# jmschrei/PyPore

Measured on AMD Instinct MI355X. Metric: Msamples/sec segmented (SpeedyStatSplit, 10^8-sample trace); %HBM roofline, higher is better.
Workload: dtype int32/f64 (exact integer block sums of fp32 or int16 samples; decisions in fp64)

## Files before the change

### pypore_amd/csrc/poreseg.hip

```cpp
#include <hip/hip_runtime.h>

#include <algorithm>
#include <chrono>
#include <complex>
#include <cmath>
#include <cstdarg>
#include <cstdio>
#include <cstdlib>
#include <cstring>
#include <initializer_list>
#include <condition_variable>
#include <mutex>
#include <string>
#include <thread>
#include <tuple>
#include <type_traits>
#include <vector>

#include "poreseg.h"
#include "seg_device.hpp"
#include "seg_align.hpp"
#include "seg_pairwise.hpp"
#include "seg_hmm.hpp"

// ... 73 lines not shown
    bool defer_sync = false;
    int scan_lds_pad = 0;
    int k0_unaligned = 1;
    int single_pass = 1;
    int gather_fused = 1;
    int download_by_kernel = 1;
    int debug = 0;
#ifdef PS_DIAG
    int dbg_phase = 0;
    int dbg_k0_nogrp = 0;
#endif
    int k0_shared = 0;
    hipEvent_t ev_front[2] = {};
    bool stream_idle = true;
    int tree_par = 1;
    int groups = 1;
    int scan_bs = 1;
    int wide_bs = 1;
    int bridge_single = 1 << 30;
    int tree_tail_pct = 0;
    int slots_pct = 100;
    int tree_jobs_per_wave = 4;
    int tree_screen = 1;
    struct OccKey { const void *fn; int nt; size_t lds; int per_cu; };
    std::vector<OccKey> occ_cache;
    std::vector<std::pair<const void *, int>> attr_cache;
    struct TileCache {
        bool valid = false;
        int32_t n_ev = 0; int mw = 0, W = 0; int64_t L = 0; bool use_bs = false;
        std::vector<int64_t> ev_start, ev_len;
        size_t nj = 0, jb = 0, up_bytes = 0; int64_t list_entries = 0, total_len = 0, sample_end = 0, nb_total = 0;
    } tile_cache;
    DevBuf bsum, ev_info, chunk_mabs, ev_boff, blk_mm, grp, filt_fwd, filt_agg, filt_zin, up_dev;
    DevBuf align_in, align_scratch;
    DevBuf pw_in, pw_scratch;
    long long pw_budget = 2ll << 30;
    DevBuf ev_info_tr;
    DevBuf blk_cls, cls_mm;
    DevBuf pre_c;
    DevBuf nt_log;
    int64_t nt_cap = 65536, nt_hdr_cap = -1;
    int64_t nt_seen = -1, nt_call_cap = 0;
    std::vector<int64_t> nt_ev_start, nt_ev_len;
    DevBuf hmm_model, hmm_off, hmm_bp, hmm_last, hmm_flags;
    std::vector<char> hmm_blob;
    long long hmm_bp_budget = 512ll << 20;
    DevBuf hmm_fmat, hmm_acc, hmm_skip;
    DevBuf hmm_pmax;
    DevBuf hmm_samp;
    long long hmm_fb_budget = 4ll << 30;
    bool hmm_expect_lds = true;
    int stitch_host = 0;
    DevBuf ev_len, det_counts, det_tics, det_cand;
    DevBuf bridges, bmeta, tile_i32, sp_off, spine_items, asm_hdr, ev_first_tile;
    DevBuf bridge_ext, ext_slot, ext_list;
    DevBuf lat_state, lat_seam, lat_res;
    unsigned lat_tag_next = 1;
    unsigned lat_tag_base = 0;
    int lat_help = 1;
    int bridge_budget = BR_MAX;
    int bridge_ext_on = 1;
    HostBuf h_hdr;
    DevBuf spine_jobs, spine_scratch, spine_dense, spine_meta, tree_jobs, tree_scratch, tree_spill, tree_defer, screen_acc,
        tree_counts, items, item_pos, first_item, ev_off, bounds_off, small;
    HostBuf h_meta, h_dense, h_small, h_up;
    hipEvent_t ev[10] = {};
    int timing = 1;
    double ms[8] = {0, 0, 0, 0, 0, 0, 0, 0};
    int64_t counters[16] = {0, 0, 0, 0, 0, 0, 0, 0, 0, 0, 0, 0, 0, 0, -1, -1};
    bool screen_ran = false;
};

namespace {

int fail(ps_ctx *ctx, int code, const char *fmt, ...)
{
    if (ctx) {
        char buf[512];
        va_list ap;
        va_start(ap, fmt);
        vsnprintf(buf, sizeof buf, fmt, ap);
        va_end(ap);
        ctx->err = buf;
    }
    return code;
}

#define HIP_TRY(ctx, expr)                                                                        \
    do {                                                                                          \
        hipError_t e_ = (expr);                                                                   \
        if (e_ != hipSuccess)                                                                     \
            return fail(ctx, PS_ERR_HIP, "%s failed: %s (%s:%d)", #expr, hipGetErrorString(e_), __FILE__, __LINE__); \
    } while (0)
// ... 36 lines not shown
        c.made = true;
    }
    const unsigned long long t = c.next++;
    *ticket = t;
    const int m = std::min(max_in_flight, K0Chain::RING / 2);
    if (t >= static_cast<unsigned long long>(m)) {
        const unsigned long long w = t - static_cast<unsigned long long>(m);
        if (c.gen[w % K0Chain::RING] == w + 1) HIP_TRY(ctx, hipStreamWaitEvent(st, c.ev[w % K0Chain::RING], 0));
    }
    return PS_OK;
}
int chain_publish(ps_ctx *ctx, int device, hipStream_t st, unsigned long long ticket)
{
    K0Chain &c = g_chain[device & 15];
    std::lock_guard<std::mutex> lk(c.mu);
    HIP_TRY(ctx, hipEventRecord(c.ev[ticket % K0Chain::RING], st));
    c.gen[ticket % K0Chain::RING] = ticket + 1;
    return PS_OK;
}
constexpr size_t SMALL_TAIL = 64 * 1024;
struct SmallLayout { unsigned long long status, work0, work1, work2, dense, stamp[12], life[9], qctl, qhead, tree_tail; AsmHeader hdr;
                     unsigned long long lat_ctl[6]; int lat_prog[LAT_D];
                     unsigned long long nt_cur;
                     unsigned long long tree_defer[3]; };

int make_cfg(ps_ctx *ctx, const void *d_samples, const ps_sample_format *fmt, int mw, int maxw, int W,
             double min_gain, DevCfg *c)
{
    if (!fmt) return fail(ctx, PS_ERR_ARG, "sample format is NULL");
    if (fmt->dtype != PS_DTYPE_F32 && fmt->dtype != PS_DTYPE_I16)
        return fail(ctx, PS_ERR_ARG, "unknown dtype %d", fmt->dtype);
    if (!(fmt->quantum > 0) || !std::isfinite(fmt->quantum))
        return fail(ctx, PS_ERR_ARG, "quantum must be positive and finite");
    c->samples = d_samples;
    c->dtype = fmt->dtype;
    c->off_counts = fmt->dtype == PS_DTYPE_F32 ? 0 : fmt->offset_counts;
    c->dc_counts = fmt->dtype == PS_DTYPE_F32 ? static_cast<double>(fmt->offset_counts) : 0.0;
    c->noise_k = ctx->noise_k;
    c->inv_q = static_cast<float>(1.0 / fmt->quantum);
    c->q = fmt->quantum;
    c->q2 = fmt->quantum * fmt->quantum;
    c->mw = mw; c->maxw = maxw; c->W = W; c->half = W / 2;
    c->min_gain = min_gain;
    c->mode = ctx->mode;
    c->prune = ctx->prune;
    c->lds_cap = std::max(1, std::min(W, ctx->lds_max_samples));
    c->bsum = nullptr; c->ev_info = nullptr; c->chunk_tot = nullptr; c->blk_mm = nullptr; c->grp = nullptr; c->bs_wide = 0;
// ... 453 lines not shown
    float ms = 0;
    if (ctx->timing >= 2 && hipEventElapsedTime(&ms, ctx->ev[2], ctx->ev[3]) == hipSuccess) ctx->ms[1] = ms;
    if (ctx->timing >= 2 && hipEventElapsedTime(&ms, ctx->ev[3], ctx->ev[4]) == hipSuccess) ctx->ms[2] = ms;
    ctx->ms[3] = std::chrono::duration<double, std::milli>(std::chrono::steady_clock::now() - t_begin).count();
    return PS_OK;
}



LatHelp lat_help_of(ps_ctx *ctx, const DevCfg &cfg, SmallLayout *sm)
{
    if (!ctx->lat_help || cfg.bsum == nullptr || !ctx->lat_res.p) return LAT_NONE;
    LatHelp h;
    h.ctl = sm->lat_ctl;
    h.state = ctx->lat_state.as<unsigned long long>();
    h.seam = ctx->lat_seam.as<int>();
    h.prog = sm->lat_prog;
    h.res = ctx->lat_res.as<unsigned long long>();
    h.tag_base = ctx->lat_tag_base;
    h.stay = ctx->lat_help == 2 ? 1 : 0;
    return h;
}

template <int DT> int launch_bridge_la(ps_ctx *ctx, const DevCfg &cfg, unsigned nj, SmallLayout *sm)
{
    const unsigned grid = std::min(nj, resident_slots(ctx, bridge_la_kernel<DT>, 64 * BR_LA, 0));
    hipLaunchKernelGGL((bridge_la_kernel<DT>), dim3(grid), dim3(64 * BR_LA), 0, ctx->stream, cfg,
                       ctx->spine_jobs.as<SpineJob>(), ctx->spine_scratch.as<int2>(), ctx->spine_meta.as<int4>(),
                       ctx->bridges.as<int2>(), ctx->bmeta.as<int4>(), reinterpret_cast<unsigned *>(&sm->status),
                       &sm->work0, static_cast<int>(nj), nullptr, nullptr, nullptr, 0, ctx->bridge_budget, static_cast<int>(EXT_MAX),
                       lat_help_of(ctx, cfg, sm));
    HIP_TRY(ctx, hipGetLastError());
    return PS_OK;
}

template <int NT, int DT> int launch_bridge(ps_ctx *ctx, const DevCfg &cfg, unsigned nj, SmallLayout *sm)
{
    ScanShape s;
    if (int rc = scan_shape<NT>(ctx, bridge_kernel<NT, DT>, cfg, nj, &s)) return rc;
    hipLaunchKernelGGL((bridge_kernel<NT, DT>), dim3(s.grid), dim3(NT), s.lds, ctx->stream, cfg,
                       ctx->spine_jobs.as<SpineJob>(), ctx->spine_scratch.as<int2>(), ctx->spine_meta.as<int4>(),
                       ctx->bridges.as<int2>(), ctx->bmeta.as<int4>(), reinterpret_cast<unsigned *>(&sm->status),
                       &sm->work0, static_cast<int>(nj), ctx->bridge_single, ctx->bridge_budget,
                       NT == 64 ? lat_help_of(ctx, cfg, sm) : LAT_NONE);
    HIP_TRY(ctx, hipGetLastError());
    return PS_OK;
}

void reset_call_stats(ps_ctx *ctx)
{
    for (double &m : ctx->ms) m = 0;
    for (int64_t &c : ctx->counters) c = 0;
    ctx->counters[14] = ctx->counters[15] = -1;
    ctx->screen_ran = false;
}

int reserve_items(ps_ctx *ctx, int64_t items_cap, int64_t total_len, int mw)
{
    const size_t n = static_cast<size_t>(std::max<int64_t>(1, items_cap));
    const size_t tscratch_bound = static_cast<size_t>(total_len / mw + items_cap + 1);
    HIP_TRY(ctx, ctx->spine_items.reserve(n * sizeof(int4)));
    HIP_TRY(ctx, ctx->tree_jobs.reserve(n * sizeof(TreeJob)));
    HIP_TRY(ctx, ctx->tree_counts.reserve((n + (static_cast<size_t>(items_cap) >> GS_LOG) + 2) * sizeof(int32_t)));
    HIP_TRY(ctx, ctx->items.reserve(n * sizeof(Item)));
    HIP_TRY(ctx, ctx->item_pos.reserve((static_cast<size_t>(items_cap) + 1) * sizeof(int64_t)));
    HIP_TRY(ctx, ctx->tree_scratch.reserve(tscratch_bound * sizeof(int32_t)));
    HIP_TRY(ctx, ctx->tree_spill.reserve(tscratch_bound * sizeof(int2)));
    if (ctx->tree_screen) {
        HIP_TRY(ctx, ctx->tree_defer.reserve(n * sizeof(int2)));
        HIP_TRY(ctx, ctx->screen_acc.reserve_zeroed(static_cast<size_t>(SCREEN_ACC) * SCREEN_ACC_STRIDE * sizeof(unsigned long long), ctx->stream));
    }
    return PS_OK;
}

struct DigestWant { bool wide = false, grp = false, blk_mm = false, cls = false; };
int reserve_digest(ps_ctx *ctx, int64_t nb_pad, int32_t n_ev, const DigestWant &want)
{
// ... 53 lines not shown
    }
    bool queued = skip_k0;
#ifdef PS_DIAG
    if constexpr (!(FLAGS & DT_WIDE)) {
        if (!queued && ns == 3) { enqueue_k0<FLAGS, 3, 6>(ctx, cfg, st, k, k0_grid, k0_grp); queued = true; }
        if (!queued && ns == 4) { enqueue_k0<FLAGS, 4, 8>(ctx, cfg, st, k, k0_grid, k0_grp); queued = true; }
    }
#endif
    if (!queued) enqueue_k0<FLAGS, 2, 2>(ctx, cfg, st, k, k0_grid, k0_grp);
    HIP_TRY(ctx, hipGetLastError());
    return PS_OK;
}
int k0_done(ps_ctx *ctx, hipStream_t st)
{
    if (!ctx->chain_held) return PS_OK;
    ctx->chain_held = false;
    return chain_publish(ctx, ctx->device, st, ctx->chain_ticket);
}

template <int FLAGS> int launch_scans_bs(ps_ctx *ctx, const DevCfg &cfg, unsigned nj, SmallLayout *sm)
{
    if (int rc = by_dtype<FLAGS>(cfg.dtype, [&](auto dt) { return launch_spine<64, dt()>(ctx, cfg, nj, sm, true); })) return rc;
    if (ctx->timing >= 2) HIP_TRY(ctx, hipEventRecord(ctx->ev[6], ctx->stream));
    if (int rc = by_dtype<FLAGS>(cfg.dtype, [&](auto dt) { return launch_bridge<64, dt()>(ctx, cfg, nj, sm); })) return rc;
    return by_dtype<FLAGS>(cfg.dtype, [&](auto dt) { return launch_bridge_la<dt()>(ctx, cfg, nj, sm); });
}

int device_stitch_batch_(ps_ctx *ctx, const DevCfg &cfg_in, int bs_mode, const int64_t *ev_start, const int64_t *ev_len, int32_t n_ev, int mw, int W,
                        int32_t *d_bounds, int64_t cap, int64_t *h_bounds_off, ps_segstat *d_stats,
                        std::chrono::steady_clock::time_point t_begin, bool digest_ready = false)
{
    DevCfg cfg = cfg_in;
    const bool use_bs = bs_mode != 0;
    const bool wide = bs_mode == 2;
    cfg.bs_wide = wide ? 1 : 0;
    int64_t L = ctx->tile_len;
    ps_ctx::TileCache &tc = ctx->tile_cache;
    const size_t evb = (static_cast<size_t>(n_ev) + 1) * sizeof(int64_t);
    bool reuse = tc.valid && tc.n_ev == n_ev && tc.mw == mw && tc.W == W && tc.L == L && tc.use_bs == use_bs &&
                 std::equal(ev_start, ev_start + n_ev, tc.ev_start.begin()) && std::equal(ev_len, ev_len + n_ev, tc.ev_len.begin());
    if (!reuse) {
        tc.valid = false;
        int64_t total_len = 0, sample_end = 0;
        for (int e = 0; e < n_ev; ++e) { total_len += ev_len[e]; sample_end = std::max(sample_end, ev_start[e] + ev_len[e]); }
        int64_t Lt = L;
        if (Lt <= 0) Lt = use_bs ? ((total_len + 4095) / 4096 >= 8LL * W ? (total_len + 4095) / 4096
                                                                         : std::max<int64_t>(4LL * W, (total_len + 1535) / 1536))
                                 : std::max<int64_t>(8LL * W, (total_len + 1023) / 1024);
// ... 39 lines not shown
    }
    const size_t nj = tc.nj, jb = tc.jb, up_bytes = tc.up_bytes;
    const int64_t list_entries = tc.list_entries, total_len = tc.total_len, sample_end = tc.sample_end;
    ctx->counters[2] = static_cast<int64_t>(nj);
    const int64_t max_items = list_entries + static_cast<int64_t>(nj) * BR_MAX;

    HIP_TRY(ctx, ctx->spine_scratch.reserve(std::max<int64_t>(1, list_entries) * sizeof(int2)));
    HIP_TRY(ctx, ctx->spine_meta.reserve(std::max<size_t>(4, nj) * sizeof(int4)));
    HIP_TRY(ctx, ctx->bridges.reserve(std::max<size_t>(1, nj) * BR_MAX * sizeof(int2)));
    if (use_bs && ctx->lat_help) {
        const size_t res_bytes = static_cast<size_t>(LAT_D) * LAT_C * sizeof(unsigned long long);
        HIP_TRY(ctx, ctx->lat_state.reserve(LAT_D * sizeof(unsigned long long)));
        HIP_TRY(ctx, ctx->lat_seam.reserve(LAT_D * sizeof(int)));
        HIP_TRY(ctx, ctx->lat_res.reserve_zeroed(res_bytes, ctx->stream));
        if (ctx->lat_tag_next + 2u * LAT_TAGS >= (1u << 24)) {
            HIP_TRY(ctx, hipMemsetAsync(ctx->lat_res.p, 0, res_bytes, ctx->stream));
            ctx->stream_idle = false;
            ctx->lat_tag_next = 1;
        }
        ctx->lat_tag_base = ctx->lat_tag_next;
        ctx->lat_tag_next += LAT_TAGS;
    }
    HIP_TRY(ctx, ctx->bmeta.reserve(std::max<size_t>(1, nj) * sizeof(int4)));
    HIP_TRY(ctx, ctx->tile_i32.reserve(std::max<size_t>(1, nj) * 4 * sizeof(int)));
    HIP_TRY(ctx, ctx->sp_off.reserve((nj + 1) * sizeof(long long)));
    if (int irc = reserve_items(ctx, max_items, total_len, mw)) return irc;
    HIP_TRY(ctx, ctx->first_item.reserve(evb));
    if (evb <= SMALL_TAIL) ctx->bounds_off.alias(ctx->small.as<char>() + sizeof(SmallLayout));
    else HIP_TRY(ctx, ctx->bounds_off.reserve(evb));
    ctx->asm_hdr.alias(&ctx->small.as<SmallLayout>()->hdr);
    HIP_TRY(ctx, ctx->h_small.reserve(sizeof(SmallLayout)));
    FrontStream *front = (ctx->k0_shared && use_bs && tc.nj) ? front_for(ctx) : nullptr;
    hipStream_t fs = front ? front->s : ctx->stream;
    std::unique_lock<std::mutex> front_lock;
    if (front) {
        front_lock = std::unique_lock<std::mutex>(front->mu);
        if (!ctx->stream_idle) {
            HIP_TRY(ctx, hipEventRecord(ctx->ev_front[0], ctx->stream));
            HIP_TRY(ctx, hipStreamWaitEvent(fs, ctx->ev_front[0], 0));
        }
    }
    {
        const char *up = ctx->h_up.as<char>();
        void *up_devptr = nullptr;
        if (ctx->upload_by_kernel && hipHostGetDevicePointer(&up_devptr, const_cast<char *>(up), 0) != hipSuccess) { up_devptr = nullptr; (void)hipGetLastError(); }
        if (up_devptr) {
// ... 121 lines not shown
            for (size_t g = 0; g < nj; ++g) n_fail += h_bm[g].w == BR_FAIL_REACHED || (h_bm[g].w == BR_FAIL && h_bm[g].x == ctx->bridge_budget);
            ext_stride = n_fail <= static_cast<size_t>(EXT_SLOTS) ? EXT_MAX : EXT_MAX_MANY;
        }
        const int slot_cap = EXT_SLOTS * (EXT_MAX / ext_stride);
        for (size_t g = 0; g < nj; ++g) {
            const bool reached = h_bm[g].w == BR_FAIL_REACHED;
            const bool gave_up = h_bm[g].x == ctx->bridge_budget;
            if (!reached && !(h_bm[g].w == BR_FAIL && gave_up)) continue;
            const bool open_tile = h_mt[g].x == 0 && h_bm[g].x == 0;
            if (!gave_up && !open_tile) { if (reached) hopeless = true; continue; }
            if (slots_used + static_cast<int>(list.size()) < slot_cap) list.push_back(static_cast<int>(g));
            else if (reached) hopeless = true;
        }
        if (list.empty() || hopeless) break;
        if (ctx->debug) fprintf(stderr, "[poreseg] second chance, round %d: %zu seams continued on the device\n", round + 1, list.size());
        const size_t n_ext = list.size();
        HIP_TRY(ctx, ctx->bridge_ext.reserve(static_cast<size_t>(EXT_SLOTS) * EXT_MAX * sizeof(int2)));
        HIP_TRY(ctx, ctx->ext_slot.reserve(nj * sizeof(int)));
        HIP_TRY(ctx, ctx->ext_list.reserve(static_cast<size_t>(EXT_SLOTS) * (EXT_MAX / EXT_MAX_MANY) * sizeof(int)));
        HIP_TRY(ctx, hipMemcpyAsync(ctx->ext_list.p, list.data(), n_ext * sizeof(int), hipMemcpyHostToDevice, ctx->stream));
        HIP_TRY(ctx, hipStreamSynchronize(ctx->stream));
        HIP_TRY(ctx, hipMemsetAsync(&sm->hdr, 0, sizeof(AsmHeader), ctx->stream));
        if (ctx->tree_screen) HIP_TRY(ctx, hipMemsetAsync(&sm->tree_defer[0], 0, sizeof sm->tree_defer[0], ctx->stream));
        {
            const unsigned g = static_cast<unsigned>(n_ext);
            auto extend = [&](auto dt) {
                hipLaunchKernelGGL((bridge_la_kernel<dt(), true>), dim3(g), dim3(64 * BR_LA), 0, ctx->stream, cfg,
                                   ctx->spine_jobs.as<SpineJob>(), ctx->spine_scratch.as<int2>(), ctx->spine_meta.as<int4>(),
                                   ctx->bridges.as<int2>(), ctx->bmeta.as<int4>(), reinterpret_cast<unsigned *>(&sm->status),
                                   &sm->work0, static_cast<int>(n_ext), ctx->ext_list.as<int>(), ctx->bridge_ext.as<int2>(),
                                   ctx->ext_slot.as<int>(), slots_used, BR_MAX, ext_stride);
            };
            if (wide) by_dtype<DT_WIDE>(cfg.dtype, extend);
            else by_dtype(cfg.dtype, extend);
            HIP_TRY(ctx, hipGetLastError());
        }
        ctx->counters[4] += static_cast<int64_t>(n_ext);
        slots_used += static_cast<int>(n_ext);
        items_cap += static_cast<int64_t>(n_ext) * ext_stride;
        if (int irc = reserve_items(ctx, items_cap, total_len, mw)) return irc;
    }
    ctx->counters[3] = hd.n_items;
    float ms = 0;
    if (ctx->timing >= 2 && nj && hipEventElapsedTime(&ms, ctx->ev[7], ctx->ev[0]) == hipSuccess) ctx->ms[6] = ms;
    if (ctx->timing >= 2 && nj && hipEventElapsedTime(&ms, ctx->ev[0], ctx->ev[6]) == hipSuccess) ctx->ms[0] = ms;
    if (ctx->timing >= 2 && nj && hipEventElapsedTime(&ms, ctx->ev[6], ctx->ev[1]) == hipSuccess) ctx->ms[5] = ms;
    if (ctx->timing >= 2 && hipEventElapsedTime(&ms, ctx->ev[1], ctx->ev[5]) == hipSuccess) ctx->ms[4] = ms;
    return rc;
}
int device_stitch_batch(ps_ctx *ctx, const DevCfg &cfg_in, int bs_mode, const int64_t *ev_start, const int64_t *ev_len, int32_t n_ev, int mw, int W,
                        int32_t *d_bounds, int64_t cap, int64_t *h_bounds_off, ps_segstat *d_stats,
                        std::chrono::steady_clock::time_point t_begin, bool digest_ready = false)
{
    const int rc = device_stitch_batch_(ctx, cfg_in, bs_mode, ev_start, ev_len, n_ev, mw, W, d_bounds, cap, h_bounds_off, d_stats, t_begin, digest_ready);
    ctx->chain_held = false;
    return rc;
}
}

namespace {
std::mutex g_probe_mu;
int g_unaligned_ok[16] = {-1, -1, -1, -1, -1, -1, -1, -1, -1, -1, -1, -1, -1, -1, -1, -1};
int k0_unaligned_probe(int device, hipStream_t st)
{
    std::lock_guard<std::mutex> lk(g_probe_mu);
// ... 98 lines not shown
        if (hipEventCreateWithFlags(&e, hipEventDisableTiming) != hipSuccess) { delete ctx; return PS_ERR_HIP; }
    if (ctx->small.reserve(sizeof(SmallLayout) + SMALL_TAIL) != hipSuccess) { delete ctx; return PS_ERR_HIP; }
    ctx->lds_max_samples = (LDS_BYTES_MAX - 1024 * 8 - 256) / (static_cast<int>(sizeof(lds_t)) + 1);
    ctx->k0_unaligned = k0_unaligned_probe(device, ctx->stream);
#ifdef PS_DIAG
    diag_env(ctx);
#endif
    *out = ctx;
    return PS_OK;
}

void ps_destroy(ps_ctx *ctx)
{
    if (!ctx) return;
    (void)hipSetDevice(ctx->device);
    (void)hipStreamSynchronize(ctx->stream);
    DevBuf *bufs[] = {&ctx->spine_jobs, &ctx->spine_scratch, &ctx->spine_dense, &ctx->spine_meta, &ctx->tree_jobs,
                      &ctx->tree_scratch, &ctx->tree_spill, &ctx->tree_defer, &ctx->screen_acc, &ctx->tree_counts, &ctx->items, &ctx->item_pos,
                      &ctx->first_item, &ctx->ev_off, &ctx->bounds_off, &ctx->small, &ctx->bridges, &ctx->bmeta,
                      &ctx->tile_i32, &ctx->sp_off, &ctx->spine_items, &ctx->asm_hdr, &ctx->ev_first_tile, &ctx->ev_len,
                      &ctx->det_counts, &ctx->det_tics, &ctx->det_cand, &ctx->bsum, &ctx->ev_info, &ctx->chunk_mabs,
                      &ctx->ev_boff, &ctx->blk_mm, &ctx->grp, &ctx->filt_fwd, &ctx->filt_agg, &ctx->filt_zin, &ctx->up_dev,
                      &ctx->align_in, &ctx->align_scratch, &ctx->pw_in, &ctx->pw_scratch, &ctx->bridge_ext, &ctx->ext_slot, &ctx->ext_list,
                      &ctx->lat_state, &ctx->lat_seam, &ctx->lat_res, &ctx->pre_c, &ctx->ev_info_tr, &ctx->blk_cls,
                      &ctx->cls_mm, &ctx->nt_log, &ctx->hmm_model, &ctx->hmm_off, &ctx->hmm_bp,
                      &ctx->hmm_last, &ctx->hmm_flags, &ctx->hmm_fmat, &ctx->hmm_acc, &ctx->hmm_skip, &ctx->hmm_pmax,
                      &ctx->hmm_samp};
    for (DevBuf *b : bufs) b->release();
    ctx->h_meta.release(); ctx->h_dense.release(); ctx->h_small.release(); ctx->h_up.release(); ctx->h_hdr.release();
    for (auto &e : ctx->ev) if (e) (void)hipEventDestroy(e);
    for (auto &e : ctx->ev_front) if (e) (void)hipEventDestroy(e);
    if (ctx->own_stream) (void)hipStreamDestroy(ctx->stream);
    delete ctx;
}

const char *ps_last_error(const ps_ctx *ctx) { return ctx ? ctx->err.c_str() : "null context"; }

int ps_set_tiling(ps_ctx *ctx, int64_t tile_len, int64_t halo)
{
    if (!ctx || tile_len < 0 || halo < 0) return PS_ERR_ARG;
    ctx->tile_len = tile_len;
    ctx->halo = halo;
    return PS_OK;
}

#ifdef PS_DIAG
static int diag_mask_stream(ps_ctx *ctx, hipStream_t *st, int first, int count, int stride, bool invert)
// ... 30 lines not shown
    else if (n == "k0_waves" && value >= 0 && value <= 16) ctx->k0_waves = static_cast<int>(value);
    else if (n == "k0_shared") ctx->k0_shared = value != 0;
    else if (n == "k0_admit" && value >= 0) ctx->k0_admit = static_cast<int>(value);
    else if (n == "bridge_ext" && (value == 0 || value == 1)) ctx->bridge_ext_on = static_cast<int>(value);
    else if (n == "lat_help" && value >= 0 && value <= 2) ctx->lat_help = static_cast<int>(value);
    else if (n == "shared_device" && value >= 0 && value <= 4096) {
        const bool sh = value > 1;
        ctx->k0_waves = sh ? 1 : 0;
        ctx->lat_help = sh ? 0 : 1;
        ctx->k0_admit = value > 3 ? 3 : 0;
    }
    else if (n == "hmm_bp_budget" && value >= 1) ctx->hmm_bp_budget = value;
    else if (n == "hmm_fb_budget" && value >= 1) ctx->hmm_fb_budget = value;
    else if (n == "pairwise_budget" && value >= 1) ctx->pw_budget = value;
    else if (n == "hmm_expect_lds") ctx->hmm_expect_lds = value != 0;
    else if (n == "single_pass") ctx->single_pass = value != 0;
    else if (n == "gather_fused") ctx->gather_fused = value != 0;
    else if (n == "download_by_kernel") ctx->download_by_kernel = value != 0;
    else if (n == "debug") ctx->debug = value != 0;
    else if (n == "k0_unaligned") ctx->k0_unaligned = value != 0 ? k0_unaligned_probe(ctx->device, ctx->stream) : 0;
    else if (n == "slots_pct" && value >= 1 && value <= 100) ctx->slots_pct = static_cast<int>(value);
    else if (n == "tree_jobs_per_wave" && value >= 0 && value <= 1024) ctx->tree_jobs_per_wave = static_cast<int>(value);
    else if (n == "tree_screen") ctx->tree_screen = value != 0;
    else if (n == "noise_k_ppm" && value >= 0) ctx->noise_k = static_cast<float>(static_cast<double>(value) * 1.0e-6);
#ifdef PS_DIAG
    else if (n == "dbg_phase" && value >= 0 && value <= 2) ctx->dbg_phase = static_cast<int>(value);
    else if (n == "dbg_k0_nogrp") ctx->dbg_k0_nogrp = value != 0;
    else if (n == "cu_mask" && ctx->own_stream)
        return diag_mask_stream(ctx, &ctx->stream, static_cast<int>(value & 0xfff), static_cast<int>((value >> 12) & 0xfff),
                                static_cast<int>((value >> 24) & 0xff), ((value >> 32) & 1) != 0);
    else if (n == "k0_sets" && value >= 2 && value <= 4) ctx->k0_sets = static_cast<int>(value);
    else if (n == "scan_lds_pad" && value >= 0 && value <= 65536) ctx->scan_lds_pad = static_cast<int>(value);
    else if (n == "rep_eval" && value >= 1) ctx->rep_eval = static_cast<int>(value);
    else if (n == "rep_stage" && value >= 1) ctx->rep_stage = static_cast<int>(value);
    else if (n == "rep_sum" && value >= 1) ctx->rep_sum = static_cast<int>(value);
#endif
    else if (n == "bridge_budget" && value >= 1 && value <= BR_MAX) ctx->bridge_budget = static_cast<int>(value);
    else if (n == "wide_bs") { ctx->wide_bs = value != 0; ctx->wide_skip = 0; }
    else if (n == "bridge_single" && value >= 1) ctx->bridge_single = static_cast<int>(value);
    else if (n == "tree_tail_pct" && value >= 0 && value <= 100) ctx->tree_tail_pct = static_cast<int>(value);
    else if (n == "filter_fused") ctx->filter_fused = value != 0;
    else if (n == "upload_by_kernel") ctx->upload_by_kernel = value != 0;
    else if (n == "timing") ctx->timing = static_cast<int>(std::max<int64_t>(0, std::min<int64_t>(2, value)));
    else if (n == "tree_mw") ctx->tree_mw = value != 0;
    else if (n == "spine_nt" && (value == 256 || value == 512 || value == 1024)) ctx->spine_nt = static_cast<int>(value);
    else if (n == "tree_nt" && (value == 256 || value == 512)) ctx->tree_nt = static_cast<int>(value);
// ... 1711 lines not shown
```

### pypore_amd/csrc/seg_device.hpp

```cpp
#pragma once
#include <hip/hip_runtime.h>
#include <stdint.h>
#include "poreseg.h"

namespace ps {

constexpr int LDS_STACK = 128;
constexpr int MAX_WAVES = 16;
constexpr int OBUF = 256;
constexpr int BR_MAX = 256;
constexpr int LST_MAX = 256;
constexpr int LAT_D = 256;
constexpr int LAT_W = 16;
constexpr int LAT_C = 2048;
constexpr int LAT_TAGS = 4096;
struct LatHelp {
    unsigned long long *ctl;
    unsigned long long *state;
    int *seam;
    int *prog;
    unsigned long long *res;
    unsigned tag_base;
    int stay;
};
// ... 1162 lines not shown
            if (threadIdx.x == 0) {
                unsigned long long pos = atomicAdd(dense_count, static_cast<unsigned long long>(cnt));
                meta[jb] = make_int4(cnt, ended, static_cast<int>(pos), 0);
                sh.bcast = static_cast<int>(pos);
            }
            __syncthreads();
            const int pos = sh.bcast;
            for (int i = threadIdx.x; i < cnt; i += NT) dense[pos + i] = i < flushed ? out[i] : sh.obuf[i - flushed];
        }
        __syncthreads();
    }
    flush(bad, wk, status, work, 0);
}

enum : int { BR_NONE = 0, BR_JOINED = 1, BR_ENDED = 2, BR_FAIL = 3, BR_DEFER = 4,
              BR_FAIL_REACHED = 5 };
__device__ __forceinline__ int2 bridge_at(const int2 *bridges, const int2 *ext, const int *ext_slot, int ext_stride, int g, int i)
{
    return i < BR_MAX ? bridges[static_cast<long long>(g) * BR_MAX + i]
                      : ext[static_cast<long long>(ext_slot[g]) * ext_stride + (i - BR_MAX)];
}
constexpr int BR_PATIENCE = 3;

template <int NT, int DT>
__global__ __launch_bounds__(NT, (NT == 64 ? PS_BRIDGE_MINW : 4)) PS_BRIDGE_REGS void bridge_kernel(DevCfg c, const SpineJob *jobs, const int2 *lists,
                                                       const int4 *meta, int2 *bridges, int4 *bmeta,
                                                       unsigned *status, unsigned long long *work, int n_jobs, int max_single,
                                                       int budget = BR_MAX,
                                                       LatHelp lat = LAT_NONE)
{
    extern __shared__ int ys[];
    __shared__ SharedT<NT> sh;
    if (c.bsum != nullptr && (*status & ST_WIDE_RANGE) != 0u) return;
    unsigned bad = 0;
    Work wk = PS_WORK_INIT;
    for (int g = blockIdx.x; g < n_jobs; g += gridDim.x) {
        const SpineJob job = jobs[g];
        const int4 m = meta[g];
        const bool last_tile = (g - job.first_tile) == job.ntiles - 1;
        if (last_tile || m.y != 0) {
            if (threadIdx.x == 0) bmeta[g] = make_int4(0, -1, 0, BR_NONE);
            continue;
        }
        if (m.x == 0 && g != job.first_tile) {
            if (threadIdx.x == 0) bmeta[g] = make_int4(0, -1, 0, BR_FAIL);
            continue;
        }
        int a = m.x > 0 ? lists[job.out_off + m.x - 1].x : job.start;
        int cnt = 0, st = BR_FAIL, jt = -1, ji = 0, cached = -1, ccnt = 0;
        const EvRef er = ev_ref_of(c, job.ev);
        for (int step = 0; step <= budget; ++step) {
            int u = a / job.tile_len;
            if (u > job.ntiles - 1) u = job.ntiles - 1;
            u += job.first_tile;
            const SpineJob uj = jobs[u];
            if (u != cached) {
                ccnt = meta[u].x;
                __syncthreads();
                for (int i = threadIdx.x; i < ccnt && i < SharedT<NT>::LN; i += NT) sh.lst[i] = lists[uj.out_off + i].x;
// ... 29 lines not shown
            bmeta[g] = make_int4(cnt, jt, ji, st);
            if (st == BR_DEFER && lat.ctl != nullptr && c.half > 0) {
                const long long ps0 = static_cast<long long>(a) + static_cast<long long>(jt + LAT_W) * c.half;
                if (ps0 < static_cast<long long>(job.end) - 2LL * c.mw) {
                    int u = static_cast<int>(ps0 / job.tile_len);
                    if (u > job.ntiles - 1) u = job.ntiles - 1;
                    const int4 mu = meta[job.first_tile + u];
                    if (mu.x == 0 && mu.y == 0) atomicAdd(&lat.ctl[0], 1ull);
                }
            }
        }
        __syncthreads();
    }
    flush(bad, wk, status, work, 1);
}

constexpr int BR_LA = 4;
template <int DT, bool EXT = false>
__global__ __launch_bounds__(64 * BR_LA, PS_BRIDGE_MINW) PS_BRIDGE_REGS void bridge_la_kernel(DevCfg c, const SpineJob *jobs, const int2 *lists,
                                                                  const int4 *meta, int2 *bridges, int4 *bmeta,
                                                                  unsigned *status, unsigned long long *work, int n_jobs,
                                                                  const int *ext_list = nullptr, int2 *ext = nullptr, int *ext_slot = nullptr,
                                                                  int slot_base = 0, int budget = BR_MAX, int ext_stride = EXT_MAX,
                                                                  LatHelp lat = LAT_NONE)
{
    __shared__ unsigned long long lat_e;
    __shared__ unsigned long long lat_state[EXT ? 1 : LAT_D];
    __shared__ int lat_prog[EXT ? 1 : LAT_D];
    __shared__ SharedT<64> shw[BR_LA];
    __shared__ int lst[LST_MAX];
    __shared__ int2 obuf[BR_MAX];
    __shared__ int2 res[BR_LA];
    if ((*status & ST_WIDE_RANGE) != 0u) return;
    const bool lat_stay = !EXT && lat.res != nullptr && c.half > 0 && (lat.ctl[0] != 0ull || lat.stay != 0);
    const int wave = __builtin_amdgcn_readfirstlane(static_cast<int>(threadIdx.x >> 6));
    SharedT<64> &sh = shw[wave];
    unsigned bad = 0;
    Work wk = PS_WORK_INIT;
    enum : int { O_CONT = 0, O_HIT = 1, O_EARLY = 2, O_LATE = 3, O_NONE = 4 };
    const int LIMIT = EXT ? BR_MAX + ext_stride : budget;
    for (int gi = blockIdx.x; gi < n_jobs; gi += gridDim.x) {
        const int g = EXT ? ext_list[gi] : gi;
        const int4 bm = bmeta[g];
        if (!EXT && bm.w != BR_DEFER) continue;
        const SpineJob job = jobs[g];
        const int4 m = meta[g];
        int cnt = bm.x;
        for (int i = threadIdx.x; i < cnt && i < BR_MAX; i += 64 * BR_LA) obuf[i] = bridges[static_cast<int64_t>(g) * BR_MAX + i];
        __syncthreads();
        const long long slot = slot_base + gi;
        int a = cnt > 0 ? obuf[cnt - 1].x : (m.x > 0 ? lists[job.out_off + m.x - 1].x : job.start);
        int st = BR_FAIL, jt = -1, ji = 0, cached = -1, ccnt = 0;
        const EvRef er = ev_ref_of(c, job.ev);
        long long jres = EXT ? (cnt == 0 && m.x == 0 ? m.z : 0) : bm.y;
        const bool lat_use = lat_stay;
        int lslot = -1;
        long long la0 = 0;
        unsigned ltag = 0;
        bool lat_valid = false;
        for (int step = cnt; step <= LIMIT; ++step) {
            int u = a / job.tile_len;
            if (u > job.ntiles - 1) u = job.ntiles - 1;
            u += job.first_tile;
            const SpineJob uj = jobs[u];
            if (u != cached) {
// ... 1156 lines not shown
```

### pypore_amd/engine.py

```python
import collections
import ctypes
import os
import threading
import warnings

import numpy as np
import torch

from . import _lib

_contexts = {}

DEFAULT_OPTIONS = {}
DEFAULT_TILING = [0, 0]
POOL_OVERRIDES = {}

EVENT_CAP = 1 << 16

_ENV_OPTIONS = {
    "PORESEG_MODE": "mode", "PORESEG_SPINE_NT": "spine_nt", "PORESEG_TREE_NT": "tree_nt", "PORESEG_PRUNE": "prune",
    "PORESEG_SCAN_BS": "scan_bs", "PORESEG_GROUPS": "groups", "PORESEG_TREE_PAR": "tree_par", "PORESEG_K0_WAVES": "k0_waves",
    "PORESEG_K0_SHARED": "k0_shared", "PORESEG_K0_MAX": "k0_admit", "PORESEG_K0_SETS": "k0_sets", "PORESEG_WIDE_BS": "wide_bs",
    "PORESEG_BRIDGE_SINGLE": "bridge_single", "PORESEG_TREE_TAIL": "tree_tail_pct", "PORESEG_FILTER_FUSED": "filter_fused",
    "PORESEG_UPLOAD": "upload_by_kernel", "PORESEG_TIMING": "timing", "PORESEG_TREE_MW": "tree_mw",
    "PORESEG_TREE_JPW": "tree_jobs_per_wave", "PORESEG_TREE_SCREEN": "tree_screen", "PORESEG_SLOTS_PCT": "slots_pct", "PORESEG_BRIDGE_EXT": "bridge_ext",
    "PORESEG_LAT_HELP": "lat_help", "PORESEG_BRIDGE_BUDGET": "bridge_budget", "PORESEG_DEBUG": "debug",
    "PORESEG_GATHER_FUSED": "gather_fused", "PORESEG_SINGLE_PASS": "single_pass", "PORESEG_DOWNLOAD": "download_by_kernel", "PORESEG_K0_UNALIGNED": "k0_unaligned",
    "PORESEG_DBG_PHASE": "dbg_phase", "PORESEG_DBG_K0_NOGRP": "dbg_k0_nogrp", "PORESEG_SCAN_LDS_PAD": "scan_lds_pad", "PORESEG_REP_STAGE": "rep_stage",
}


def options_from_env(environ=None):
    env = os.environ if environ is None else environ
    opts = {}
    for var, name in _ENV_OPTIONS.items():
        if var in env and env[var] != "":
            opts[name] = int(env[var])
    if env.get("PORESEG_STITCH"):
        opts["stitch_host"] = 1 if env["PORESEG_STITCH"] == "host" else 0
    if "PORESEG_NOISE_K" in env:
        opts["noise_k_ppm"] = int(round(float(env["PORESEG_NOISE_K"]) * 1e6))
    tiling = [int(env.get("PORESEG_TILE", "0") or 0), int(env.get("PORESEG_HALO", "0") or 0)]
    pool = {}
    if "PORESEG_POOL_K0_WAVES" in env:
        pool["k0_waves"] = int(env["PORESEG_POOL_K0_WAVES"])
    if "PORESEG_POOL_K0_MAX" in env:
        pool["k0_admit"] = int(env["PORESEG_POOL_K0_MAX"])
    if env.get("PORESEG_POOL_SHARED", "0") == "1":
# ... 899 lines not shown
```

Baseline: 537,300.

## Add seam-join prepass that resolves easy tile seams before bridge kernels

Adds a lightweight seam_join_kernel that, for each tile seam, classifies it as none, failed, or directly joinable by binary-searching the next tile's split list for the current endpoint. Joined and trivial seams get their bmeta written immediately, and only unresolved seams are compacted into a list. The bridge and lookahead-bridge kernels then iterate over that compacted list instead of every job, and the bridge grid shrinks accordingly. This saves scanning work on seams that need no bridging, at the cost of an extra launch, an atomic-based compaction, and a counter reset on the extension path.

Measured after the change: 534,600. No clear change (-0.5%).

```diff
diff --git a/pypore_amd/csrc/poreseg.hip b/pypore_amd/csrc/poreseg.hip
--- a/pypore_amd/csrc/poreseg.hip
+++ b/pypore_amd/csrc/poreseg.hip
@@ -119,6 +119,7 @@
     int slots_pct = 100;
     int tree_jobs_per_wave = 4;
     int tree_screen = 1;
+    int seam_join = 1;
     struct OccKey { const void *fn; int nt; size_t lds; int per_cu; };
     std::vector<OccKey> occ_cache;
     std::vector<std::pair<const void *, int>> attr_cache;
@@ -151,6 +152,7 @@
     DevBuf ev_len, det_counts, det_tics, det_cand;
     DevBuf bridges, bmeta, tile_i32, sp_off, spine_items, asm_hdr, ev_first_tile;
     DevBuf bridge_ext, ext_slot, ext_list;
+    DevBuf seam_list;
     DevBuf lat_state, lat_seam, lat_res;
     unsigned lat_tag_next = 1;
     unsigned lat_tag_base = 0;
@@ -166,6 +168,7 @@
     double ms[8] = {0, 0, 0, 0, 0, 0, 0, 0};
     int64_t counters[16] = {0, 0, 0, 0, 0, 0, 0, 0, 0, 0, 0, 0, 0, 0, -1, -1};
     bool screen_ran = false;
+    bool join_ran = false;
 };
 
 namespace {
@@ -248,7 +251,8 @@
 struct SmallLayout { unsigned long long status, work0, work1, work2, dense, stamp[12], life[9], qctl, qhead, tree_tail; AsmHeader hdr;
                      unsigned long long lat_ctl[6]; int lat_prog[LAT_D];
                      unsigned long long nt_cur;
-                     unsigned long long tree_defer[3]; };
+                     unsigned long long tree_defer[3];
+                     unsigned long long seam_join[JOIN_CTL]; };
 
 int make_cfg(ps_ctx *ctx, const void *d_samples, const ps_sample_format *fmt, int mw, int maxw, int W,
              double min_gain, DevCfg *c)
@@ -748,29 +752,43 @@
     return h;
 }
 
-template <int DT> int launch_bridge_la(ps_ctx *ctx, const DevCfg &cfg, unsigned nj, SmallLayout *sm)
+template <int DT> int launch_bridge_la(ps_ctx *ctx, const DevCfg &cfg, unsigned nj, SmallLayout *sm, bool listed = false)
 {
     const unsigned grid = std::min(nj, resident_slots(ctx, bridge_la_kernel<DT>, 64 * BR_LA, 0));
     hipLaunchKernelGGL((bridge_la_kernel<DT>), dim3(grid), dim3(64 * BR_LA), 0, ctx->stream, cfg,
                        ctx->spine_jobs.as<SpineJob>(), ctx->spine_scratch.as<int2>(), ctx->spine_meta.as<int4>(),
                        ctx->bridges.as<int2>(), ctx->bmeta.as<int4>(), reinterpret_cast<unsigned *>(&sm->status),
-                       &sm->work0, static_cast<int>(nj), nullptr, nullptr, nullptr, 0, ctx->bridge_budget, static_cast<int>(EXT_MAX),
-                       lat_help_of(ctx, cfg, sm));
+                       &sm->work0, static_cast<int>(nj), listed ? ctx->seam_list.as<int>() : nullptr, nullptr, nullptr, 0,
+                       ctx->bridge_budget, static_cast<int>(EXT_MAX), lat_help_of(ctx, cfg, sm), listed ? &sm->seam_join[0] : nullptr);
     HIP_TRY(ctx, hipGetLastError());
     return PS_OK;
 }
 
-template <int NT, int DT> int launch_bridge(ps_ctx *ctx, const DevCfg &cfg, unsigned nj, SmallLayout *sm)
+template <int NT, int DT> int launch_bridge(ps_ctx *ctx, const DevCfg &cfg, unsigned nj, SmallLayout *sm, bool listed = false)
 {
     ScanShape s;
     if (int rc = scan_shape<NT>(ctx, bridge_kernel<NT, DT>, cfg, nj, &s)) return rc;
+    if (listed) s.grid = std::max(1u, std::min(s.grid, (nj + 3) / 4));
     hipLaunchKernelGGL((bridge_kernel<NT, DT>), dim3(s.grid), dim3(NT), s.lds, ctx->stream, cfg,
                        ctx->spine_jobs.as<SpineJob>(), ctx->spine_scratch.as<int2>(), ctx->spine_meta.as<int4>(),
                        ctx->bridges.as<int2>(), ctx->bmeta.as<int4>(), reinterpret_cast<unsigned *>(&sm->status),
                        &sm->work0, static_cast<int>(nj), ctx->bridge_single, ctx->bridge_budget,
-                       NT == 64 ? lat_help_of(ctx, cfg, sm) : LAT_NONE);
+                       NT == 64 ? lat_help_of(ctx, cfg, sm) : LAT_NONE,
+                       listed ? ctx->seam_list.as<int>() : nullptr, listed ? &sm->seam_join[0] : nullptr);
     HIP_TRY(ctx, hipGetLastError());
     return PS_OK;
+}
+
+bool launch_seam_join(ps_ctx *ctx, unsigned nj, SmallLayout *sm)
+{
+    if (!ctx->seam_join || ctx->seam_list.cap < nj * sizeof(int)) return false;
+    const unsigned grid = std::min((nj + JOIN_NT - 1) / JOIN_NT, 1024u);
+    hipLaunchKernelGGL(seam_join_kernel, dim3(grid), dim3(JOIN_NT), 0, ctx->stream, ctx->spine_jobs.as<SpineJob>(),
+                       ctx->spine_scratch.as<int2>(), ctx->spine_meta.as<int4>(), ctx->bmeta.as<int4>(),
+                       reinterpret_cast<const unsigned *>(&sm->status), static_cast<int>(nj), ctx->seam_list.as<int>(), sm->seam_join);
+    if (hipGetLastError() != hipSuccess) return false;
+    ctx->join_ran = true;
+    return true;
 }
 
 void reset_call_stats(ps_ctx *ctx)
@@ -779,6 +797,7 @@
     for (int64_t &c : ctx->counters) c = 0;
     ctx->counters[14] = ctx->counters[15] = -1;
     ctx->screen_ran = false;
+    ctx->join_ran = false;
 }
 
 int reserve_items(ps_ctx *ctx, int64_t items_cap, int64_t total_len, int mw)
@@ -878,8 +897,9 @@
 {
     if (int rc = by_dtype<FLAGS>(cfg.dtype, [&](auto dt) { return launch_spine<64, dt()>(ctx, cfg, nj, sm, true); })) return rc;
     if (ctx->timing >= 2) HIP_TRY(ctx, hipEventRecord(ctx->ev[6], ctx->stream));
-    if (int rc = by_dtype<FLAGS>(cfg.dtype, [&](auto dt) { return launch_bridge<64, dt()>(ctx, cfg, nj, sm); })) return rc;
-    return by_dtype<FLAGS>(cfg.dtype, [&](auto dt) { return launch_bridge_la<dt()>(ctx, cfg, nj, sm); });
+    const bool listed = launch_seam_join(ctx, nj, sm);
+    if (int rc = by_dtype<FLAGS>(cfg.dtype, [&](auto dt) { return launch_bridge<64, dt()>(ctx, cfg, nj, sm, listed); })) return rc;
+    return by_dtype<FLAGS>(cfg.dtype, [&](auto dt) { return launch_bridge_la<dt()>(ctx, cfg, nj, sm, listed); });
 }
 
 int device_stitch_batch_(ps_ctx *ctx, const DevCfg &cfg_in, int bs_mode, const int64_t *ev_start, const int64_t *ev_len, int32_t n_ev, int mw, int W,
@@ -965,6 +985,7 @@
         ctx->lat_tag_next += LAT_TAGS;
     }
     HIP_TRY(ctx, ctx->bmeta.reserve(std::max<size_t>(1, nj) * sizeof(int4)));
+    if (use_bs && ctx->seam_join) HIP_TRY(ctx, ctx->seam_list.reserve(std::max<size_t>(1, nj) * sizeof(int)));
     HIP_TRY(ctx, ctx->tile_i32.reserve(std::max<size_t>(1, nj) * 4 * sizeof(int)));
     HIP_TRY(ctx, ctx->sp_off.reserve((nj + 1) * sizeof(long long)));
     if (int irc = reserve_items(ctx, max_items, total_len, mw)) return irc;
@@ -1132,6 +1153,7 @@
         HIP_TRY(ctx, hipStreamSynchronize(ctx->stream));
         HIP_TRY(ctx, hipMemsetAsync(&sm->hdr, 0, sizeof(AsmHeader), ctx->stream));
         if (ctx->tree_screen) HIP_TRY(ctx, hipMemsetAsync(&sm->tree_defer[0], 0, sizeof sm->tree_defer[0], ctx->stream));
+        if (ctx->join_ran) HIP_TRY(ctx, hipMemsetAsync(&sm->seam_join[0], 0, sizeof sm->seam_join[0], ctx->stream));
         {
             const unsigned g = static_cast<unsigned>(n_ext);
             auto extend = [&](auto dt) {
@@ -1151,6 +1173,10 @@
         if (int irc = reserve_items(ctx, items_cap, total_len, mw)) return irc;
     }
     ctx->counters[3] = hd.n_items;
+    if (ctx->debug && ctx->join_ran && (rc == PS_OK || rc == RC_FALLBACK)) {
+        const unsigned long long *sj = ctx->h_small.as<SmallLayout>()->seam_join;
+        fprintf(stderr, "[poreseg] seam join: %zu seams, %llu joined, %llu none, %llu failed, %llu listed\n", nj, sj[1], sj[2], sj[3], sj[4]);
+    }
     float ms = 0;
     if (ctx->timing >= 2 && nj && hipEventElapsedTime(&ms, ctx->ev[7], ctx->ev[0]) == hipSuccess) ctx->ms[6] = ms;
     if (ctx->timing >= 2 && nj && hipEventElapsedTime(&ms, ctx->ev[0], ctx->ev[6]) == hipSuccess) ctx->ms[0] = ms;
@@ -1295,7 +1321,7 @@
                       &ctx->det_counts, &ctx->det_tics, &ctx->det_cand, &ctx->bsum, &ctx->ev_info, &ctx->chunk_mabs,
                       &ctx->ev_boff, &ctx->blk_mm, &ctx->grp, &ctx->filt_fwd, &ctx->filt_agg, &ctx->filt_zin, &ctx->up_dev,
                       &ctx->align_in, &ctx->align_scratch, &ctx->pw_in, &ctx->pw_scratch, &ctx->bridge_ext, &ctx->ext_slot, &ctx->ext_list,
-                      &ctx->lat_state, &ctx->lat_seam, &ctx->lat_res, &ctx->pre_c, &ctx->ev_info_tr, &ctx->blk_cls,
+                      &ctx->seam_list, &ctx->lat_state, &ctx->lat_seam, &ctx->lat_res, &ctx->pre_c, &ctx->ev_info_tr, &ctx->blk_cls,
                       &ctx->cls_mm, &ctx->nt_log, &ctx->hmm_model, &ctx->hmm_off, &ctx->hmm_bp,
                       &ctx->hmm_last, &ctx->hmm_flags, &ctx->hmm_fmat, &ctx->hmm_acc, &ctx->hmm_skip, &ctx->hmm_pmax,
                       &ctx->hmm_samp};
@@ -1372,6 +1398,7 @@
     else if (n == "slots_pct" && value >= 1 && value <= 100) ctx->slots_pct = static_cast<int>(value);
     else if (n == "tree_jobs_per_wave" && value >= 0 && value <= 1024) ctx->tree_jobs_per_wave = static_cast<int>(value);
     else if (n == "tree_screen") ctx->tree_screen = value != 0;
+    else if (n == "seam_join") ctx->seam_join = value != 0;
     else if (n == "noise_k_ppm" && value >= 0) ctx->noise_k = static_cast<float>(static_cast<double>(value) * 1.0e-6);
 #ifdef PS_DIAG
     else if (n == "dbg_phase" && value >= 0 && value <= 2) ctx->dbg_phase = static_cast<int>(value);
diff --git a/pypore_amd/csrc/seg_device.hpp b/pypore_amd/csrc/seg_device.hpp
--- a/pypore_amd/csrc/seg_device.hpp
+++ b/pypore_amd/csrc/seg_device.hpp
@@ -1208,19 +1208,83 @@
 }
 constexpr int BR_PATIENCE = 3;
 
+#ifndef PS_JOIN_VGPRS
+#define PS_JOIN_VGPRS 32
+#endif
+constexpr int JOIN_NT = 256;
+constexpr int JOIN_CTL = 6;
+__global__ __launch_bounds__(JOIN_NT) __attribute__((amdgpu_num_vgpr(PS_JOIN_VGPRS))) void seam_join_kernel(
+    const SpineJob *__restrict__ jobs, const int2 *__restrict__ lists, const int4 *__restrict__ meta, int4 *__restrict__ bmeta,
+    const unsigned *status, int n_jobs, int *__restrict__ seam_list, unsigned long long *ctl)
+{
+    if ((*status & ST_WIDE_RANGE) != 0u) return;
+    enum : int { J_IDLE = -1, J_LIST = -2 };
+    const int lane = static_cast<int>(threadIdx.x & 63u);
+    for (int g0 = blockIdx.x * JOIN_NT; g0 < n_jobs; g0 += gridDim.x * JOIN_NT) {
+        const int g = g0 + static_cast<int>(threadIdx.x);
+        int st = J_IDLE;
+        if (g < n_jobs) {
+            const SpineJob job = jobs[g];
+            const int4 m = meta[g];
+            const bool last_tile = (g - job.first_tile) == job.ntiles - 1;
+            if (last_tile || m.y != 0) st = BR_NONE;
+            else if (m.x == 0 && g != job.first_tile) st = BR_FAIL;
+            else {
+                const int a = m.x > 0 ? lists[job.out_off + m.x - 1].x : job.start;
+                int u = a / job.tile_len;
+                if (u > job.ntiles - 1) u = job.ntiles - 1;
+                u += job.first_tile;
+                int found = -2;
+                if (a == jobs[u].start) found = -1;
+                else {
+                    const int2 *lu = lists + jobs[u].out_off;
+                    int lo = 0, hi = meta[u].x - 1;
+                    while (lo <= hi) {
+                        const int mid = (lo + hi) >> 1;
+                        const int v = lu[mid].x;
+                        if (v == a) { found = mid; break; }
+                        if (v < a) lo = mid + 1; else hi = mid - 1;
+                    }
+                }
+                if (found != -2 && u != g) { st = BR_JOINED; bmeta[g] = make_int4(0, u, found, BR_JOINED); }
+                else st = J_LIST;
+            }
+            if (st == BR_NONE || st == BR_FAIL) bmeta[g] = make_int4(0, -1, 0, st);
+        }
+        const unsigned long long listed = __ballot(st == J_LIST);
+        const int n_joined = __popcll(__ballot(st == BR_JOINED)), n_none = __popcll(__ballot(st == BR_NONE)),
+                  n_fail = __popcll(__ballot(st == BR_FAIL)), n_list = __popcll(listed);
+        unsigned long long base = 0;
+        if (lane == 0) {
+            if (n_list) { base = atomicAdd(&ctl[0], static_cast<unsigned long long>(n_list)); atomicAdd(&ctl[4], static_cast<unsigned long long>(n_list)); }
+            if (n_joined) atomicAdd(&ctl[1], static_cast<unsigned long long>(n_joined));
+            if (n_none) atomicAdd(&ctl[2], static_cast<unsigned long long>(n_none));
+            if (n_fail) atomicAdd(&ctl[3], static_cast<unsigned long long>(n_fail));
+        }
+        if (n_list) {
+            base = __shfl(base, 0);
+            if (st == J_LIST) seam_list[base + __popcll(listed & ((1ull << lane) - 1ull))] = g;
+        }
+    }
+}
+
 template <int NT, int DT>
 __global__ __launch_bounds__(NT, (NT == 64 ? PS_BRIDGE_MINW : 4)) PS_BRIDGE_REGS void bridge_kernel(DevCfg c, const SpineJob *jobs, const int2 *lists,
                                                        const int4 *meta, int2 *bridges, int4 *bmeta,
                                                        unsigned *status, unsigned long long *work, int n_jobs, int max_single,
                                                        int budget = BR_MAX,
-                                                       LatHelp lat = LAT_NONE)
+                                                       LatHelp lat = LAT_NONE,
+                                                       const int *seam_list = nullptr, const unsigned long long *seam_count = nullptr)
 {
     extern __shared__ int ys[];
     __shared__ SharedT<NT> sh;
     if (c.bsum != nullptr && (*status & ST_WIDE_RANGE) != 0u) return;
     unsigned bad = 0;
     Work wk = PS_WORK_INIT;
-    for (int g = blockIdx.x; g < n_jobs; g += gridDim.x) {
+    const bool listed = NT == 64 && seam_list != nullptr;
+    const int n_seams = listed ? min(static_cast<int>(*seam_count), n_jobs) : n_jobs;
+    for (int gi = blockIdx.x; gi < n_seams; gi += gridDim.x) {
+        const int g = listed ? seam_list[gi] : gi;
         const SpineJob job = jobs[g];
         const int4 m = meta[g];
         const bool last_tile = (g - job.first_tile) == job.ntiles - 1;
@@ -1296,7 +1360,8 @@
                                                                   unsigned *status, unsigned long long *work, int n_jobs,
                                                                   const int *ext_list = nullptr, int2 *ext = nullptr, int *ext_slot = nullptr,
                                                                   int slot_base = 0, int budget = BR_MAX, int ext_stride = EXT_MAX,
-                                                                  LatHelp lat = LAT_NONE)
+                                                                  LatHelp lat = LAT_NONE,
+                                                                  const unsigned long long *seam_count = nullptr)
 {
     __shared__ unsigned long long lat_e;
     __shared__ unsigned long long lat_state[EXT ? 1 : LAT_D];
@@ -1314,7 +1379,11 @@
     enum : int { O_CONT = 0, O_HIT = 1, O_EARLY = 2, O_LATE = 3, O_NONE = 4 };
     const int LIMIT = EXT ? BR_MAX + ext_stride : budget;
     for (int gi = blockIdx.x; gi < n_jobs; gi += gridDim.x) {
-        const int g = EXT ? ext_list[gi] : gi;
+        int g = EXT ? ext_list[gi] : gi;
+        if (!EXT && seam_count != nullptr) {
+            if (gi >= static_cast<int>(*seam_count)) break;
+            g = ext_list[gi];
+        }
         const int4 bm = bmeta[g];
         if (!EXT && bm.w != BR_DEFER) continue;
         const SpineJob job = jobs[g];
diff --git a/pypore_amd/engine.py b/pypore_amd/engine.py
--- a/pypore_amd/engine.py
+++ b/pypore_amd/engine.py
@@ -23,7 +23,7 @@
     "PORESEG_K0_SHARED": "k0_shared", "PORESEG_K0_MAX": "k0_admit", "PORESEG_K0_SETS": "k0_sets", "PORESEG_WIDE_BS": "wide_bs",
     "PORESEG_BRIDGE_SINGLE": "bridge_single", "PORESEG_TREE_TAIL": "tree_tail_pct", "PORESEG_FILTER_FUSED": "filter_fused",
     "PORESEG_UPLOAD": "upload_by_kernel", "PORESEG_TIMING": "timing", "PORESEG_TREE_MW": "tree_mw",
-    "PORESEG_TREE_JPW": "tree_jobs_per_wave", "PORESEG_TREE_SCREEN": "tree_screen", "PORESEG_SLOTS_PCT": "slots_pct", "PORESEG_BRIDGE_EXT": "bridge_ext",
+    "PORESEG_TREE_JPW": "tree_jobs_per_wave", "PORESEG_TREE_SCREEN": "tree_screen", "PORESEG_SEAM_JOIN": "seam_join", "PORESEG_SLOTS_PCT": "slots_pct", "PORESEG_BRIDGE_EXT": "bridge_ext",
     "PORESEG_LAT_HELP": "lat_help", "PORESEG_BRIDGE_BUDGET": "bridge_budget", "PORESEG_DEBUG": "debug",
     "PORESEG_GATHER_FUSED": "gather_fused", "PORESEG_SINGLE_PASS": "single_pass", "PORESEG_DOWNLOAD": "download_by_kernel", "PORESEG_K0_UNALIGNED": "k0_unaligned",
     "PORESEG_DBG_PHASE": "dbg_phase", "PORESEG_DBG_K0_NOGRP": "dbg_k0_nogrp", "PORESEG_SCAN_LDS_PAD": "scan_lds_pad", "PORESEG_REP_STAGE": "rep_stage",
```
